# irconde/SSL4POLYP

Hardware: AMD Instinct MI355X
Metric: training-step images/sec/node, ViT-B/16 224^2 (cls fine-tune) (higher is better)
Workload: dtype bf16; 1 GPU; ViT-B/16 classification fine-tune, bs=64/GPU, 224^2, AdamW, random init, finetune mode full (finetune.py:49-91); global_batch=64, parallelism=dp1, launch=eager, lr_schedule=constant

## Files before the change

include/polypmae.h:

```cpp
#ifndef POLYPMAE_H
#define POLYPMAE_H
#include <stddef.h>
#include <stdint.h>

#ifdef __cplusplus
extern "C" {
#endif

enum pm_status { PM_OK = 0, PM_EINVAL = -1, PM_ESHAPE = -2, PM_EARCH = -3, PM_ELAUNCH = -4, PM_EALIGN = -5 };
enum pm_dtype { PM_F32 = 0, PM_BF16 = 1, PM_F16 = 2 };

enum pm_epilogue {
  PM_EPI_STORE = 0,
  PM_EPI_GELU = 1,
  PM_EPI_RESIDUAL = 2,
  PM_EPI_DGELU = 3,
  PM_EPI_ACCUM = 4
};

const char* pm_strerror(int status);
int pm_abi_version(void);

int pm_layernorm_fwd(const float* x, long ldx, const float* gamma, const float* beta, void* y, int out_dtype,
                     float* mean, float* rstd, int M, int D, float eps, void* stream);
// ... 172 lines not shown
                            size_t ws_bytes, void* stream);

typedef struct pm_block_fwd_desc {
  const float* x;
  float* x_mid;
  float* x_out;
  void* ln1;
  float* mean1;
  float* rstd1;
  void* qkv;
  float* lse;
  void* attn;
  void* ln2;
  float* mean2;
  float* rstd2;
  void* h_pre;
  void* h_act;
  const float *norm1_w, *norm1_b, *norm2_w, *norm2_b;
  const void *qkv_w, *proj_w, *fc1_w, *fc2_w;
  const float *qkv_b, *proj_b, *fc1_b, *fc2_b;
  int rows, samples, N, D, Hd, heads;
  int dtype;
  int gemm_variant;
  float eps;
} pm_block_fwd_desc;
int pm_vit_block_fwd(const pm_block_fwd_desc* d, void* stream);

typedef struct pm_block_bwd_desc {
  const float* x_in;
  const float* x_mid;
  const void *ln1, *qkv, *attn, *ln2, *h_pre, *h_act;
  const float *mean1, *rstd1, *mean2, *rstd2, *lse;
  const float *norm1_w, *norm2_w;
  const void *qkv_w, *proj_w, *fc1_w, *fc2_w;
  const float* dx;
  const void* dx_act;
  float* dmid;
  void* dmid_act;
  float* din;
  void* din_act;
  void *d_hidden, *d_qkv, *d_ln, *d_attn;
  float* delta;
  float *g_norm1_w, *g_norm1_b, *g_norm2_w, *g_norm2_b;
  float *g_qkv_w, *g_proj_w, *g_fc1_w, *g_fc2_w;
  float *g_qkv_b, *g_proj_b, *g_fc1_b, *g_below_bias;
  void* ws_ln;
  size_t ws_ln_bytes;
  void* ws_group;
  size_t ws_group_bytes;
  void *side_stream, *ev_join, *ev_fork, *ev_done;
  int samples, N, D, Hd, heads, dtype, gemm_variant, group_blocks, accumulate;
  int two_groups;
  void *side_stream2, *ev_fork2, *ev_done2;
} pm_block_bwd_desc;
int pm_vit_block_bwd(const pm_block_bwd_desc* d, void* stream);

int pm_vit_head_fwd(const float* x, int N, int pool, const float* gamma, const float* beta, const float* W,
                    const float* bias, float* feat, float* xhat_mean, float* mean, float* rstd, float* logits, int B, int D,
                    int n_class, float eps, void* stream);
int pm_vit_head_bwd(const float* dlogits, const float* dfeat, const float* x, int N, int pool, const float* gamma,
                    const float* W, const float* feat, const float* xhat_mean, const float* mean, const float* rstd,
                    float* dx, void* dx_act, int act_dtype, float* dW, float* dbias, float* dgamma, float* dbeta, int B,
                    int D, int n_class, void* stream);
int pm_cls_head_fwd(const float* x, int N, const float* gamma, const float* beta, const float* W, const float* bias,
                    float* xn, float* mean, float* rstd, float* logits, int B, int D, int n_class, float eps,
                    void* stream);
int pm_cls_head_bwd(const float* dlogits, const float* x, int N, const float* gamma, const float* W, const float* xn,
                    const float* mean, const float* rstd, float* dx, void* dx_act, int act_dtype, float* dW,
                    float* dbias, float* dgamma, float* dbeta, int B, int D, int n_class, void* stream);

int pm_supervised_loss_fwd(const float* logits, const long long* targets, const float* pos_weight,
                           const float* class_weights, float* loss, float* dlogits, int B, int n_class, void* stream);
int pm_scale(const float* x, const float* scale, float* out, long n, void* stream);

int pm_dgelu(const void* dy, const void* pre, void* out, int dtype, long n, void* stream);

int pm_adamw(float* p, const float* g, float* m, float* v, void* shadow, int shadow_dtype, long n, float lr,
             float beta1, float beta2, float eps, float weight_decay, int step, float grad_scale, void* stream);

int pm_adamw_tick(float* hyper, int n_groups, void* stream);
int pm_adamw_dev(float* p, const float* g, float* m, float* v, void* shadow, int shadow_dtype, long n,
                 const float* hyper, void* stream);

int pm_loss_scale_update(float* state, const float* stats, float* hyper, int n_groups, float growth_factor,
                         float backoff_factor, int growth_interval, void* stream);

int pm_grad_stats(const float* g, long n, float* out, void* stream);

enum pm_ws_kind { PM_WS_LAYERNORM_BWD = 1, PM_WS_COLSUM = 2, PM_WS_UNSHUFFLE_BWD = 4 };
size_t pm_gemm_workspace_bytes(int a_kmajor, int b_kmajor, int in_dtype, int M, int N, int K, const pm_gemm_opts* opts);
size_t pm_workspace_bytes(int kind, int M, int N);

typedef struct pm_comm pm_comm;
int pm_comm_unique_id(void* id128);
int pm_comm_create(pm_comm** out, const void* id128, int rank, int world);
int pm_comm_world(const pm_comm* c, int* rank, int* world);
int pm_comm_allreduce_f32(pm_comm* c, float* base, const long* lo, const long* hi, int n_buckets, void* stream);
int pm_comm_destroy(pm_comm* c);

int pm_boot_metrics_workspace(int N, int M, int R, int K, int C, size_t* bytes);
int pm_boot_metrics(const double* score, const int* order, const unsigned char* label, const int* cluster, const int* draws,
                    const double* tau, double* out, int N, int M, int R, int K, int C, int sorted_ready, void* workspace,
                    size_t ws_bytes, void* stream);

int pm_select_tau_workspace(int N, int M, size_t* bytes);
int pm_select_tau(const double* score, const int* order, const unsigned char* label, const double* previous_tau, int policy,
                  double* out, double* candidates, int N, int M, void* workspace, size_t ws_bytes, void* stream);

#ifdef __cplusplus
}
#endif
#endif
```

ssl4polyp_amd/_lib.py:

```python
from __future__ import annotations

import ctypes
import os
from ctypes import c_char_p, c_float, c_int, c_long, c_void_p

PM_F32, PM_BF16, PM_F16 = 0, 1, 2
EPI_STORE, EPI_GELU, EPI_RESIDUAL, EPI_DGELU, EPI_ACCUM = 0, 1, 2, 3, 4

_HERE = os.path.dirname(os.path.abspath(__file__))
LIB_PATH = os.environ.get("POLYPMAE_LIB") or os.path.join(_HERE, "lib", "libpolypmae.so")

P, I, L, F = c_void_p, c_int, c_long, c_float

SIGNATURES = {
    "pm_layernorm_fwd": [P, L, P, P, P, I, P, P, I, I, F, P],
    "pm_layernorm_bwd": [P, I, P, L, P, P, P, P, L, P, L, P, I, P, P, P, I, I, P, ctypes.c_size_t, P],
    "pm_vit_block_fwd": [P, P],
    "pm_vit_block_bwd": [P, P],
    "pm_gemm": [P, L, I, P, L, I, I, P, P, L, I, I, P, P, I, I, I, P],
    "pm_gemm_ws": [P, L, I, P, L, I, I, P, P, L, I, I, P, P, I, I, I, P, ctypes.c_size_t, P],
    "pm_gemm_ex": [P, L, I, P, L, I, I, P, P, L, I, I, P, P, I, I, I, P, ctypes.c_size_t, P, P],
    "pm_wgrad_group": [P, I, I, I, I, P, ctypes.c_size_t, P],
    "pm_wgrad_group_plan": [P, I, I, I, P, P, P],
    "pm_gemm_plan": [I, I, I, I, I, I, I, I, I, I, ctypes.c_size_t, P, P],
    "pm_attention_plan": [I, I, I, I, I, I, P],
    "pm_attention_fwd": [P, P, P, I, I, I, I, I, P],
    "pm_attention_bwd": [P, P, P, P, P, P, I, I, I, I, I, P],
    "pm_colsum": [P, L, I, P, I, I, P],
    "pm_colsum_ws": [P, L, I, P, I, I, P, ctypes.c_size_t, P],
    "pm_patch_im2col": [P, P, P, L, I, I, I, I, I, I, P],
    "pm_pad_cast": [P, L, P, L, I, I, I, I, I, P],
    "pm_unpad_add": [P, L, P, L, I, I, I, P],
    "pm_assemble_tokens": [P, P, P, P, P, I, I, I, P],
    "pm_assemble_tokens_bwd": [P, P, P, I, P, P, I, I, I, P],
    "pm_mae_noise": [P, L, ctypes.c_ulonglong, ctypes.c_uint, P],
    "pm_mae_masking": [P, P, P, P, I, I, I, P],
    "pm_mae_unshuffle": [P, P, P, P, P, I, I, I, I, P],
    "pm_mae_unshuffle_bwd": [P, P, P, I, P, I, I, I, I, P, ctypes.c_size_t, P],
    "pm_mae_loss_fwd": [P, P, L, I, P, I, I, I, I, I, P],
    "pm_mae_loss_finish": [P, P, L, P, P, P],
    "pm_mae_loss_bwd": [P, P, L, I, P, P, P, P, L, I, I, I, I, I, I, P],
    "pm_cast": [P, P, I, L, P],
    "pm_gather_rows": [P, L, P, P, I, L, P],
    "pm_scatter_rows_zero": [P, P, P, I, L, P],
    "pm_preprocess_u8": [P, P, P, I, I, I, F, F, F, F, F, F, P],
    "pm_aug_resize_u8": [P, P, P, P, P, I, P, P, I, I, I, I, I, I, P],
    "pm_aug_resized_crop_u8": [P, P, P, I, I, I, I, I, P, ctypes.c_size_t, P],
    "pm_aug_resized_crop_ragged_u8": [P, P, P, P, P, I, I, I, I, I, P, ctypes.c_size_t, P],
    "pm_aug_color_jitter_u8": [P, P, P, P, I, I, I, P],
    "pm_aug_gaussian_blur_u8": [P, P, P, P, I, I, I, I, P],
    "pm_aug_geometry_u8": [P, P, P, I, I, I, I, F, F, F, F, F, F, P],
    "pm_aug_pil_gaussian_blur_u8": [P, P, P, P, I, I, I, I, P],
    "pm_aug_occlude_u8": [P, P, I, I, I, P],
    "pm_aug_jpeg_roundtrip_u8": [P, P, P, I, I, I, P],
    "pm_jpeg_decode": [P, L, P, I, P, I, P, I, P, I, P, L, P, I, P, P, L, L, P, L, P],
    "pm_jpeg_decode_parallel": [P, L, P, I, P, I, P, I, P, I, P, L, P, I, P, P, L, L, P, L, P, I, I, P, ctypes.c_size_t, P, P],
    "pm_jpeg_decode_workspace": [I, I, P],
    "pm_jpeg_decode_planes": [P, L, P, I, P, I, P, I, P, I, P, P, L, P, I, I, P, ctypes.c_size_t, P, P],
    "pm_jpeg_resized_crop_workspace": [I, I, I, I, P],
    "pm_jpeg_resized_crop_u8": [P, L, P, I, P, L, P, I, P, P, P, P, I, I, I, I, I, P, ctypes.c_size_t, P],
    "pm_comm_unique_id": [P],
    "pm_comm_create": [P, P, I, I],
    "pm_comm_world": [P, P, P],
    "pm_comm_allreduce_f32": [P, P, P, P, I, P],
    "pm_comm_destroy": [P],
    "pm_vit_head_fwd": [P, I, I, P, P, P, P, P, P, P, P, P, I, I, I, F, P],
    "pm_vit_head_bwd": [P, P, P, I, I, P, P, P, P, P, P, P, P, I, P, P, P, P, I, I, I, P],
    "pm_supervised_loss_fwd": [P, P, P, P, P, P, I, I, P],
    "pm_scale": [P, P, P, L, P],
    "pm_cls_head_fwd": [P, I, P, P, P, P, P, P, P, P, I, I, I, F, P],
    "pm_cls_head_bwd": [P, P, I, P, P, P, P, P, P, P, I, P, P, P, P, I, I, I, P],
    "pm_adamw": [P, P, P, P, P, I, L, F, F, F, F, F, I, F, P],
    "pm_adamw_tick": [P, I, P],
    "pm_adamw_dev": [P, P, P, P, P, I, L, P, P],
    "pm_grad_stats": [P, L, P, P],
    "pm_loss_scale_update": [P, P, P, I, F, F, I, P],
    "pm_dgelu": [P, P, P, I, L, P],
    "pm_boot_metrics_workspace": [I, I, I, I, I, P],
    "pm_boot_metrics": [P, P, P, P, P, P, P, I, I, I, I, I, I, P, ctypes.c_size_t, P],
    "pm_select_tau_workspace": [I, I, P],
    "pm_select_tau": [P, P, P, P, I, P, P, I, I, P, ctypes.c_size_t, P],
}

ABI_VERSION = 16
PM_GROUP_WHOLE_K = -1

WS_LAYERNORM_BWD, WS_COLSUM, WS_UNSHUFFLE_BWD = 1, 2, 4


class GemmPlanInfo(ctypes.Structure):
    _fields_ = [("family", c_int), ("cfg", c_int), ("tile_m", c_int), ("tile_n", c_int), ("split_k", c_int), ("band", c_int),
                ("ws_bytes", ctypes.c_size_t)]


GEMM_GENERIC, GEMM_LDS128, GEMM_RING, GEMM_RING_WGRAD = 0, 1, 2, 3


class AttentionPlanInfo(ctypes.Structure):
    _fields_ = [("family", c_int), ("nt", c_int), ("ct", c_int), ("grid", c_int), ("launches", c_int),
                ("lds_bytes", ctypes.c_size_t * 2)]


ATTN_FWD_HEAD, ATTN_FWD_PERSISTENT, ATTN_BWD_SPLIT, ATTN_BWD_FUSED = 0, 1, 2, 3


class GemmOpts(ctypes.Structure):
    _fields_ = [("max_blocks", c_int), ("variant", c_int)]


class WgradItem(ctypes.Structure):
    _fields_ = [("dY", c_void_p), ("lddy", c_long), ("X", c_void_p), ("ldx", c_long), ("dW", c_void_p), ("lddw", c_long),
                ("n_out", c_int), ("n_in", c_int), ("accumulate", c_int), ("dbias", c_void_p)]


class BlockBwdDesc(ctypes.Structure):
    _fields_ = ([(n, c_void_p) for n in ("x_in", "x_mid", "ln1", "qkv", "attn", "ln2", "h_pre", "h_act", "mean1", "rstd1", "mean2",
                                        "rstd2", "lse", "norm1_w", "norm2_w", "qkv_w", "proj_w", "fc1_w", "fc2_w", "dx", "dx_act",
                                        "dmid", "dmid_act", "din", "din_act", "d_hidden", "d_qkv", "d_ln", "d_attn", "delta",
                                        "g_norm1_w", "g_norm1_b", "g_norm2_w", "g_norm2_b", "g_qkv_w", "g_proj_w", "g_fc1_w",
                                        "g_fc2_w", "g_qkv_b", "g_proj_b", "g_fc1_b", "g_below_bias")] +
                [("ws_ln", c_void_p), ("ws_ln_bytes", ctypes.c_size_t), ("ws_group", c_void_p), ("ws_group_bytes", ctypes.c_size_t)] +
                [(n, c_void_p) for n in ("side_stream", "ev_join", "ev_fork", "ev_done")] +
                [(n, c_int) for n in ("samples", "N", "D", "Hd", "heads", "dtype", "gemm_variant", "group_blocks", "accumulate",
                                      "two_groups")] +
                [(n, c_void_p) for n in ("side_stream2", "ev_fork2", "ev_done2")])


class BlockFwdDesc(ctypes.Structure):
    _fields_ = ([(n, c_void_p) for n in ("x", "x_mid", "x_out", "ln1", "mean1", "rstd1", "qkv", "lse", "attn", "ln2", "mean2",
                                        "rstd2", "h_pre", "h_act", "norm1_w", "norm1_b", "norm2_w", "norm2_b", "qkv_w", "proj_w",
                                        "fc1_w", "fc2_w", "qkv_b", "proj_b", "fc1_b", "fc2_b")] +
                [(n, c_int) for n in ("rows", "samples", "N", "D", "Hd", "heads", "dtype", "gemm_variant")] +
                [("eps", ctypes.c_float)])


PM_EINVAL, PM_ESHAPE, PM_EALIGN = -1, -2, -5
_lib = None


class PolypMaeError(RuntimeError):
    pass


def load():
    global _lib
    if _lib is not None:
        return _lib
    if not os.path.exists(LIB_PATH):
        raise PolypMaeError(
            f"{LIB_PATH} not found: build it with `python -c 'import __graft_entry__ as g; g.build()'`. "
            "There is no CPU/eager fallback for the MI355X hot path.")
    lib = ctypes.CDLL(LIB_PATH)
    lib.pm_strerror.restype = c_char_p
    lib.pm_strerror.argtypes = [c_int]
    lib.pm_abi_version.restype = c_int
    lib.pm_abi_version.argtypes = []
    if lib.pm_abi_version() != ABI_VERSION:
        raise PolypMaeError(f"{LIB_PATH} has ABI version {lib.pm_abi_version()}, this package binds version {ABI_VERSION}: "
                            "rebuild with `python -c 'import __graft_entry__ as g; g.build(force=True)'`")
    lib.pm_gemm_workspace_bytes.restype = ctypes.c_size_t
    lib.pm_gemm_workspace_bytes.argtypes = [I, I, I, I, I, I, P]
    lib.pm_workspace_bytes.restype = ctypes.c_size_t
    lib.pm_workspace_bytes.argtypes = [I, I, I]
    lib.pm_aug_resized_crop_workspace_bytes.restype = ctypes.c_size_t
    lib.pm_aug_resized_crop_workspace_bytes.argtypes = [I, I, I, I]
    lib.pm_wgrad_group_workspace_bytes.restype = ctypes.c_size_t
    lib.pm_wgrad_group_workspace_bytes.argtypes = [P, I, I, I]
    for name, argtypes in SIGNATURES.items():
        fn = getattr(lib, name)
        fn.restype = c_int
        fn.argtypes = argtypes
    _lib = lib
    return lib


def check(status: int, what: str) -> None:
    if status != 0:
        raise PolypMaeError(f"{what} failed: {load().pm_strerror(status).decode()} (status {status})")


def dtype_code(torch_dtype) -> int:
    import torch

    if torch_dtype == torch.float32:
        return PM_F32
    if torch_dtype == torch.bfloat16:
        return PM_BF16
    if torch_dtype == torch.float16:
        return PM_F16
    raise PolypMaeError(f"unsupported dtype {torch_dtype}")
```

ssl4polyp_amd/csrc/pm_misc.hip:

```cpp
#include "pm_common.h"

namespace {

template <typename T>
__global__ __launch_bounds__(256) void colsum_kernel(const T* __restrict__ x, long ldx, float* __restrict__ out,
                                                     float* __restrict__ partials, int M, int N) {
  const int lane = threadIdx.x & 63, wave = threadIdx.x >> 6;
  const int n = blockIdx.x * 256 + lane * 4;
  f32x4 acc = {0.f, 0.f, 0.f, 0.f};
  if (n < N) {
    for (long m = (long)blockIdx.y * 4 + wave; m < M; m += (long)gridDim.y * 4) acc += load4<T>(x + m * ldx + n);
  }
  block_colsum_tail(acc, out, partials, N);
}

template <typename T>
__global__ __launch_bounds__(256) void im2col_kernel(const float* __restrict__ imgs, const int* __restrict__ ids_keep,
                                                     T* __restrict__ cols, long ldcols, int C, int img, int p, int keep) {
  const int b = blockIdx.x / keep, j = blockIdx.x % keep;
  const int grid = img / p;
  const int pid = ids_keep ? ids_keep[b * keep + j] : j;
  const int gy = pid / grid, gx = pid % grid;
  const float* src = imgs + (long)b * C * img * img + (long)gy * p * img + gx * p;
  T* dst = cols + (long)blockIdx.x * ldcols;
// ... 118 lines not shown
                                                            int B, int H, int W, f32x4 mean, f32x4 stdv) {
  const int w4 = W >> 2;
  const long total = (long)B * H * w4;
  for (long id = (long)blockIdx.x * 256 + threadIdx.x; id < total; id += (long)gridDim.x * 256) {
    const int xq = id % w4;
    const int y = (id / w4) % H;
    const int b = id / ((long)w4 * H);
    const int f = flags ? flags[b] : 0;
    const int sy = (f & 2) ? H - 1 - y : y;
    const unsigned char* row = src + ((long)b * H + sy) * W * 3;
    float px[4][3];
#pragma unroll
    for (int i = 0; i < 4; ++i) {
      const int x = xq * 4 + i;
      const int sx = (f & 1) ? W - 1 - x : x;
#pragma unroll
      for (int c = 0; c < 3; ++c) px[i][c] = (float)row[sx * 3 + c];
    }
#pragma unroll
    for (int c = 0; c < 3; ++c) {
      f32x4 v;
#pragma unroll
      for (int i = 0; i < 4; ++i) v[i] = __fdiv_rn(__fdiv_rn(px[i][c], 255.0f) - mean[c], stdv[c]);
      *reinterpret_cast<f32x4*>(dst + (((long)b * 3 + c) * H + y) * W + xq * 4) = v;
    }
  }
}

template <typename T>
__global__ __launch_bounds__(256) void cast_kernel(const float* __restrict__ src, T* __restrict__ dst, long n) {
  const long nvec = n >> 2;
  for (long i = (long)blockIdx.x * 256 + threadIdx.x; i < nvec; i += (long)gridDim.x * 256)
    store4<T>(dst + 4 * i, *reinterpret_cast<const f32x4*>(src + 4 * i));
  if (blockIdx.x == 0 && threadIdx.x < (n & 3)) dst[(nvec << 2) + threadIdx.x] = (T)src[(nvec << 2) + threadIdx.x];
}

template <typename T>
__global__ __launch_bounds__(256) void dgelu_kernel(const T* __restrict__ dy, const T* __restrict__ pre, T* __restrict__ out, long n) {
  const long nvec = n >> 2;
  for (long i = (long)blockIdx.x * 256 + threadIdx.x; i < nvec; i += (long)gridDim.x * 256)
    store4<T>(out + 4 * i, load4<T>(dy + 4 * i) * gelu_act_grad4<T>(load4<T>(pre + 4 * i)));
}

template <typename T>
__global__ __launch_bounds__(256) void adamw_kernel(float* __restrict__ p, const float* __restrict__ g, float* __restrict__ m,
                                                    float* __restrict__ v, T* __restrict__ shadow, long n, float lr,
                                                    float beta1, float beta2, float eps, float wd, float bc1, float rsqrt_bc2,
                                                    float gscale) {
  const long nvec = n >> 2;
  for (long i = (long)blockIdx.x * 256 + threadIdx.x; i < nvec; i += (long)gridDim.x * 256) {
    f32x4 pp = *reinterpret_cast<const f32x4*>(p + 4 * i);
    const f32x4 gg = *reinterpret_cast<const f32x4*>(g + 4 * i);
    f32x4 mm = *reinterpret_cast<const f32x4*>(m + 4 * i);
    f32x4 vv = *reinterpret_cast<const f32x4*>(v + 4 * i);
#pragma unroll
    for (int e = 0; e < 4; ++e) {
      const float gr = gg[e] * gscale;
      pp[e] *= (1.0f - lr * wd);
      mm[e] = beta1 * mm[e] + (1.0f - beta1) * gr;
      vv[e] = beta2 * vv[e] + (1.0f - beta2) * gr * gr;
      const float denom = sqrtf(vv[e]) * rsqrt_bc2 + eps;
      pp[e] -= (lr / bc1) * (mm[e] / denom);
    }
    *reinterpret_cast<f32x4*>(p + 4 * i) = pp;
    *reinterpret_cast<f32x4*>(m + 4 * i) = mm;
    *reinterpret_cast<f32x4*>(v + 4 * i) = vv;
    if (shadow) store4<T>(shadow + 4 * i, pp);
  }
}


constexpr int kHyperStride = 16;
__global__ void adamw_tick_kernel(float* __restrict__ hyper, int n_groups) {
  const int g = blockIdx.x * blockDim.x + threadIdx.x;
  if (g >= n_groups) return;
  float* h = hyper + (long)g * kHyperStride;
  if (h[9] != 0.f) return;
  const float step = h[6] + 1.0f;
  h[6] = step;
  h[7] = (float)(1.0 - pow((double)h[1], (double)step));
  h[8] = (float)(1.0 / sqrt(1.0 - pow((double)h[2], (double)step)));
}

template <typename T>
__global__ __launch_bounds__(256) void adamw_dev_kernel(float* __restrict__ p, const float* __restrict__ g, float* __restrict__ m,
                                                        float* __restrict__ v, T* __restrict__ shadow, long n,
                                                        const float* __restrict__ hyper) {
  if (hyper[9] != 0.f) return;
  const float lr = hyper[0], beta1 = hyper[1], beta2 = hyper[2], eps = hyper[3], wd = hyper[4];
  const float gscale = hyper[5] * (hyper[10] != 0.f ? hyper[10] : 1.0f);
  const float bc1 = hyper[7], rsqrt_bc2 = hyper[8];
  const long nvec = n >> 2;
  for (long i = (long)blockIdx.x * 256 + threadIdx.x; i < nvec; i += (long)gridDim.x * 256) {
    f32x4 pp = *reinterpret_cast<const f32x4*>(p + 4 * i);
    const f32x4 gg = *reinterpret_cast<const f32x4*>(g + 4 * i);
    f32x4 mm = *reinterpret_cast<const f32x4*>(m + 4 * i);
    f32x4 vv = *reinterpret_cast<const f32x4*>(v + 4 * i);
#pragma unroll
    for (int e = 0; e < 4; ++e) {
      const float gr = gg[e] * gscale;
      pp[e] *= (1.0f - lr * wd);
      mm[e] = beta1 * mm[e] + (1.0f - beta1) * gr;
      vv[e] = beta2 * vv[e] + (1.0f - beta2) * gr * gr;
      const float denom = sqrtf(vv[e]) * rsqrt_bc2 + eps;
      pp[e] -= (lr / bc1) * (mm[e] / denom);
    }
    *reinterpret_cast<f32x4*>(p + 4 * i) = pp;
    *reinterpret_cast<f32x4*>(m + 4 * i) = mm;
    *reinterpret_cast<f32x4*>(v + 4 * i) = vv;
    if (shadow) store4<T>(shadow + 4 * i, pp);
  }
}

__global__ __launch_bounds__(256) void grad_stats_kernel(const float* __restrict__ g, long n, float* __restrict__ out) {
  __shared__ float red[3][4];
  float ss = 0.f, nn = 0.f, ni = 0.f;
  const long nvec = n >> 2;
  for (long i = (long)blockIdx.x * 256 + threadIdx.x; i < nvec; i += (long)gridDim.x * 256) {
    const f32x4 v = *reinterpret_cast<const f32x4*>(g + 4 * i);
#pragma unroll
    for (int e = 0; e < 4; ++e) {
      ss += v[e] * v[e];
      nn += (v[e] != v[e]) ? 1.f : 0.f;
      ni += (fabsf(v[e]) == INFINITY) ? 1.f : 0.f;
    }
  }
  if (blockIdx.x == 0 && threadIdx.x < (n & 3)) {
    const float v = g[(nvec << 2) + threadIdx.x];
    ss += v * v;
    nn += (v != v) ? 1.f : 0.f;
    ni += (fabsf(v) == INFINITY) ? 1.f : 0.f;
  }
  ss = wave_sum(ss);
  nn = wave_sum(nn);
  ni = wave_sum(ni);
  const int lane = threadIdx.x & 63, wave = threadIdx.x >> 6;
  if (lane == 0) {
    red[0][wave] = ss;
    red[1][wave] = nn;
    red[2][wave] = ni;
  }
  __syncthreads();
  if (threadIdx.x < 3) {
    const int k = threadIdx.x;
    atomicAdd(out + k, (red[k][0] + red[k][1]) + (red[k][2] + red[k][3]));
  }
}

__global__ void loss_scale_update_kernel(float* __restrict__ state, const float* __restrict__ stats, float* __restrict__ hyper,
                                         int n_groups, float growth, float backoff, int interval) {
  const float scale = state[0];
  const float found = (stats[1] + stats[2]) > 0.f ? 1.f : 0.f;
  const float tracker = state[1];
  __syncthreads();
  for (int g = threadIdx.x; g < n_groups; g += blockDim.x) {
    hyper[(long)g * kHyperStride + 9] = found;
    hyper[(long)g * kHyperStride + 10] = 1.0f / scale;
  }
  if (threadIdx.x == 0) {
    state[2] = found;
    state[4] += 1.f;
    state[5] = 1.0f / scale;
    if (found != 0.f) {
      state[0] = scale * backoff;
      state[1] = 0.f;
      state[3] += 1.f;
    } else {
      const float t = tracker + 1.f;
      if (t >= (float)interval) {
        state[0] = scale * growth;
        state[1] = 0.f;
      } else {
        state[1] = t;
      }
    }
  }
}

__global__ __launch_bounds__(256) void gather_rows_kernel(const unsigned int* __restrict__ src, long ld_words, const int* __restrict__ idx,
                                                          unsigned int* __restrict__ dst, int R, long words) {
  const long total = (long)R * words;
  for (long i = (long)blockIdx.x * 256 + threadIdx.x; i < total; i += (long)gridDim.x * 256) {
    const int r = i / words;
    const long w = i % words;
    dst[i] = src[(long)idx[r] * ld_words + w];
  }
}
__global__ __launch_bounds__(256) void scatter_rows_zero_kernel(const u32x4* __restrict__ src, const int* __restrict__ inv,
                                                                u32x4* __restrict__ dst, int M, long vecs) {
  const long total = (long)M * vecs;
  for (long i = (long)blockIdx.x * 256 + threadIdx.x; i < total; i += (long)gridDim.x * 256) {
    const int m = i / vecs;
    const long v = i % vecs;
// ... 75 lines not shown
                                                   (T*)demb, dpos, B, keep, D));
  if (dcls)
    hipLaunchKernelGGL(cls_grad_kernel, dim3((D + 63) / 64), dim3(256), 0, pm_stream(stream), dx, dcls, dpos, B,
                       (long)(keep + 1) * D, D);
  return pm_check_launch();
}

extern "C" int pm_preprocess_u8(const unsigned char* src, const unsigned char* flip_flags, float* dst, int B, int H, int W,
                                float mean_r, float mean_g, float mean_b, float std_r, float std_g, float std_b,
                                void* stream) {
  if (!src || !dst) return PM_EINVAL;
  if (B <= 0 || H <= 0 || W <= 0 || (W & 3)) return PM_ESHAPE;
  if (((uintptr_t)dst & 15)) return PM_EALIGN;
  if (!(std_r > 0.f) || !(std_g > 0.f) || !(std_b > 0.f)) return PM_EINVAL;
  const long total = (long)B * H * (W >> 2);
  const dim3 grid(cap_grid(total, 256, 8192));
  hipLaunchKernelGGL(preprocess_u8_kernel, grid, dim3(256), 0, pm_stream(stream), src, flip_flags, dst, B, H, W,
                     f32x4{mean_r, mean_g, mean_b, 0.f}, f32x4{std_r, std_g, std_b, 1.f});
  return pm_check_launch();
}

extern "C" int pm_cast(const float* src, void* dst, int dst_dtype, long n, void* stream) {
  if (!src || !dst) return PM_EINVAL;
  if (n <= 0) return PM_ESHAPE;
  if (((uintptr_t)src & 15) || ((uintptr_t)dst & 7)) return PM_EALIGN;
  const dim3 grid(cap_grid(n >> 2, 256, 4096));
  PM_DISPATCH_ACT(dst_dtype, T, hipLaunchKernelGGL(cast_kernel<T>, grid, dim3(256), 0, pm_stream(stream), src, (T*)dst, n));
  return pm_check_launch();
}

extern "C" int pm_gather_rows(const void* src, long ld_bytes, const int* idx, void* dst, int R, long row_bytes, void* stream) {
  if (!src || !idx || !dst) return PM_EINVAL;
  if (R <= 0 || row_bytes <= 0 || ld_bytes < row_bytes) return PM_ESHAPE;
  if ((row_bytes & 3) || (ld_bytes & 3) || ((uintptr_t)src & 3) || ((uintptr_t)dst & 3)) return PM_EALIGN;
  const long total = (long)R * (row_bytes >> 2);
  hipLaunchKernelGGL(gather_rows_kernel, dim3(cap_grid(total, 256, 4096)), dim3(256), 0, pm_stream(stream), (const unsigned int*)src,
                     ld_bytes >> 2, idx, (unsigned int*)dst, R, row_bytes >> 2);
  return pm_check_launch();
}

extern "C" int pm_scatter_rows_zero(const void* src, const int* inv, void* dst, int M, long row_bytes, void* stream) {
  if (!src || !inv || !dst) return PM_EINVAL;
  if (M <= 0 || row_bytes <= 0) return PM_ESHAPE;
  if ((row_bytes & 15) || ((uintptr_t)src & 15) || ((uintptr_t)dst & 15)) return PM_EALIGN;
  const long total = (long)M * (row_bytes >> 4);
  hipLaunchKernelGGL(scatter_rows_zero_kernel, dim3(cap_grid(total, 256, 8192)), dim3(256), 0, pm_stream(stream), (const u32x4*)src, inv,
                     (u32x4*)dst, M, row_bytes >> 4);
  return pm_check_launch();
}

extern "C" int pm_dgelu(const void* dy, const void* pre, void* out, int dtype, long n, void* stream) {
  if (!dy || !pre || !out) return PM_EINVAL;
  if (n <= 0 || (n & 3)) return PM_ESHAPE;
  if (((uintptr_t)dy & 7) || ((uintptr_t)pre & 7) || ((uintptr_t)out & 7)) return PM_EALIGN;
  const dim3 grid(cap_grid(n >> 2, 256, 4096));
  PM_DISPATCH_ACT(dtype, T, hipLaunchKernelGGL(dgelu_kernel<T>, grid, dim3(256), 0, pm_stream(stream), (const T*)dy, (const T*)pre,
                                               (T*)out, n));
  return pm_check_launch();
}

extern "C" int pm_adamw(float* p, const float* g, float* m, float* v, void* shadow, int shadow_dtype, long n, float lr,
                        float beta1, float beta2, float eps, float weight_decay, int step, float grad_scale,
                        void* stream) {
  if (!p || !g || !m || !v) return PM_EINVAL;
  if (n <= 0 || (n & 3) || step < 1) return PM_ESHAPE;
  const double bc1 = 1.0 - pow((double)beta1, (double)step);
  const double bc2 = 1.0 - pow((double)beta2, (double)step);
  const float rsqrt_bc2 = (float)(1.0 / sqrt(bc2));
  const dim3 grid(cap_grid(n >> 2, 256, 4096));
  if (!shadow) shadow_dtype = PM_BF16;
  PM_DISPATCH_ACT(shadow_dtype, T, hipLaunchKernelGGL(adamw_kernel<T>, grid, dim3(256), 0, pm_stream(stream), p, g, m, v, (T*)shadow, n,
                                                      lr, beta1, beta2, eps, weight_decay, (float)bc1, rsqrt_bc2, grad_scale));
  return pm_check_launch();
}


extern "C" int pm_adamw_tick(float* hyper, int n_groups, void* stream) {
  if (!hyper) return PM_EINVAL;
  if (n_groups <= 0) return PM_ESHAPE;
  hipLaunchKernelGGL(adamw_tick_kernel, dim3((n_groups + 63) / 64), dim3(64), 0, pm_stream(stream), hyper, n_groups);
  return pm_check_launch();
}

extern "C" int pm_adamw_dev(float* p, const float* g, float* m, float* v, void* shadow, int shadow_dtype, long n,
                            const float* hyper, void* stream) {
  if (!p || !g || !m || !v || !hyper) return PM_EINVAL;
  if (n <= 0 || (n & 3)) return PM_ESHAPE;
  const dim3 grid(cap_grid(n >> 2, 256, 4096));
  if (!shadow) shadow_dtype = PM_BF16;
  PM_DISPATCH_ACT(shadow_dtype, T, hipLaunchKernelGGL(adamw_dev_kernel<T>, grid, dim3(256), 0, pm_stream(stream), p, g, m, v, (T*)shadow,
                                                      n, hyper));
  return pm_check_launch();
}

extern "C" int pm_loss_scale_update(float* state, const float* stats, float* hyper, int n_groups, float growth_factor,
                                    float backoff_factor, int growth_interval, void* stream) {
  if (!state || !stats || !hyper) return PM_EINVAL;
  if (n_groups <= 0 || growth_interval <= 0 || !(growth_factor >= 1.f) || !(backoff_factor > 0.f && backoff_factor <= 1.f)) return PM_ESHAPE;
  hipLaunchKernelGGL(loss_scale_update_kernel, dim3(1), dim3(64), 0, pm_stream(stream), state, stats, hyper, n_groups,
                     growth_factor, backoff_factor, growth_interval);
  return pm_check_launch();
}

extern "C" int pm_grad_stats(const float* g, long n, float* out, void* stream) {
  if (!g || !out) return PM_EINVAL;
  if (n <= 0) return PM_ESHAPE;
  if ((uintptr_t)g & 15) return PM_EALIGN;
  hipLaunchKernelGGL(grad_stats_kernel, dim3(cap_grid(n >> 2, 256, 1024)), dim3(256), 0, pm_stream(stream), g, n, out);
  return pm_check_launch();
}

extern "C" const char* pm_strerror(int status) {
  switch (status) {
    case PM_OK: return "ok";
    case PM_EINVAL: return "invalid argument (null pointer / unknown dtype or epilogue)";
    case PM_ESHAPE: return "unsupported shape";
    case PM_EARCH: return "no gfx950 device";
    case PM_ELAUNCH: return "kernel launch failed";
    case PM_EALIGN: return "pointer / leading dimension not 16-byte aligned";
    default: return "unknown status";
  }
}

extern "C" int pm_abi_version(void) { return 16; }

extern "C" size_t pm_workspace_bytes(int kind, int M, int N) {
  if (M <= 0 || N <= 0) return 0;
  switch (kind) {
    case PM_WS_LAYERNORM_BWD: {
      long g = (M + 3) / 4;
      if (g > 1024) g = 1024;
      if (g < 64) g = 64;
      return (size_t)g * 3 * N * sizeof(float);
    }
    case PM_WS_COLSUM: return (size_t)cap_grid(M, 64, 128) * N * sizeof(float);
    case PM_WS_UNSHUFFLE_BWD: return (size_t)1024 * N * sizeof(float);
    default: return 0;
  }
}
```

ssl4polyp_amd/optim.py:

```python
from __future__ import annotations

from typing import Dict, Iterable, List, Optional

import contextlib

import torch

from . import _lib
from .engine import _ptr, _stream


def add_weight_decay(model, weight_decay=1e-5, skip_list=()):
    decay, no_decay = [], []
    for name, param in model.named_parameters():
        if not param.requires_grad:
            continue
        if len(param.shape) == 1 or name.endswith(".bias") or name in skip_list:
            no_decay.append(param)
        else:
            decay.append(param)
    return [{"params": no_decay, "weight_decay": 0.0}, {"params": decay, "weight_decay": weight_decay}]


class FusedAdamW(torch.optim.Optimizer):
# ... 45 lines not shown
        segs = []
        for r, lo, hi in items:
            if segs and segs[-1][0] == r and segs[-1][2] == lo:
                segs[-1] = (r, segs[-1][1], hi)
            else:
                segs.append((r, lo, hi))
        return segs

    HYPER_STRIDE = 16

    def _host_hyper(self):
        rows = []
        for group in self.param_groups:
            b1, b2 = group["betas"]
            rows.append((float(group["lr"]), float(b1), float(b2), float(group["eps"]), float(group["weight_decay"]),
                         float(self.grad_scale)))
        return rows

    def sync_hyper(self, force: bool = False):
        f = self._ensure_state()
        rows = self._host_hyper()
        if getattr(self, "_hyper", None) is None or self._hyper.device != f.device:
            self._hyper = torch.zeros(len(rows), self.HYPER_STRIDE, dtype=torch.float32, device=f.device)
            for gi, group in enumerate(self.param_groups):
                self._hyper[gi, 6] = float(group.get("step", 0))
            self._hyper_host = None
        if force or rows != self._hyper_host:
            if f.device.type == "cuda":
                if getattr(self, "_hyper_pin", None) is None or self._hyper_pin[0].shape[0] != len(rows):
                    self._hyper_pin = [torch.empty(len(rows), 6, dtype=torch.float32).pin_memory() for _ in range(4)]
                    self._hyper_pin_ev = [None] * 4
                    self._hyper_slot = 0
                i = self._hyper_slot
                self._hyper_slot = (i + 1) % 4
                if self._hyper_pin_ev[i] is not None:
                    self._hyper_pin_ev[i].synchronize()
                self._hyper_pin[i].copy_(torch.tensor(rows, dtype=torch.float32))
                self._hyper[:, :6].copy_(self._hyper_pin[i], non_blocking=True)
                ev = torch.cuda.Event()
                ev.record(torch.cuda.current_stream(f.device))
                self._hyper_pin_ev[i] = ev
            else:
                self._hyper[:, :6].copy_(torch.tensor(rows, dtype=torch.float32))
            self._hyper_host = rows

    @torch.no_grad()
    def step(self, closure=None, loss_scaler: "Optional[LossScaler]" = None):
        loss = None
        if closure is not None:
            with torch.enable_grad():
                loss = closure()
        f = self._ensure_state()
        rt = self._rt
        rt.wait_updates()
        if self.grad_sync is not None:
            self.grad_sync.wait()
        capturing = f.device.type == "cuda" and torch.cuda.is_current_stream_capturing()
        if not capturing or getattr(self, "_hyper", None) is None:
            self.sync_hyper()
        lib = self._rt.k.lib
        overlap = self.overlap_forward and not capturing and f.device.type == "cuda"
        work = []
        for gi, group in enumerate(self.param_groups):
            group["step"] = int(group.get("step", 0)) + 1
            for r, lo, hi in self._segments(f, group):
                work.append((gi, r, lo, hi))
        scaled = loss_scaler is not None and loss_scaler.enabled
        stat_segs = [(r, lo, hi) for _, r, lo, hi in work] if scaled else []
        if not scaled and getattr(self, "_scaler_used", False):
            self._hyper[:, 9:11] = 0.0
            self._scaler_used = False
        if overlap:
            cuts = sorted(f.offset[i] for i, n in enumerate(f.names) if n.endswith("attn.qkv.weight"))
            split = []
            for gi, r, lo, hi in work:
                if r != "mat":
                    split.append((gi, r, lo, hi))
                    continue
                pts = [lo] + [c for c in cuts if lo < c < hi] + [hi]
                split += [(gi, r, a, b) for a, b in zip(pts[:-1], pts[1:])]
            work = sorted(split, key=lambda w: (w[1] != "vec", w[2]))
            main = torch.cuda.current_stream(f.device)
            side = rt.k.side_stream(f.device)
            ev = torch.cuda.Event()
            ev.record(main)
            side.wait_event(ev)
            stream_ctx = torch.cuda.stream(side)
        else:
            stream_ctx = contextlib.nullcontext()
        with stream_ctx:
            if scaled:
                state, stats = loss_scaler._device_state(f.device)
                stats.zero_()
                for r, lo, hi in stat_segs:
                    _lib.check(lib.pm_grad_stats(_ptr(f.G[r][lo:hi]), hi - lo, _ptr(stats), _stream()), "pm_grad_stats")
                _lib.check(lib.pm_loss_scale_update(_ptr(state), _ptr(stats), _ptr(self._hyper), len(self.param_groups),
                                                    loss_scaler.growth_factor, loss_scaler.backoff_factor,
                                                    loss_scaler.growth_interval, _stream()), "pm_loss_scale_update")
                self._scaler_used = True
            _lib.check(lib.pm_adamw_tick(_ptr(self._hyper), len(self.param_groups), _stream()), "pm_adamw_tick")
            for gi, r, lo, hi in work:
                shadow = f.S[lo:hi] if (r == "mat" and f.S is not None) else None
                _lib.check(lib.pm_adamw_dev(_ptr(f.P[r][lo:hi]), _ptr(f.G[r][lo:hi]), _ptr(self._M[r][lo:hi]),
                                            _ptr(self._V[r][lo:hi]), _ptr(shadow),
                                            _lib.dtype_code(shadow.dtype) if shadow is not None else 0, hi - lo,
                                            _ptr(self._hyper[gi]), _stream()), "pm_adamw_dev")
                if overlap:
                    done = torch.cuda.Event()
                    done.record(side)
                    rt.pending_updates.append((r, lo, hi, done))
        return loss

    def sync(self) -> None:
        self._rt.wait_updates()

    def grad_stats(self) -> torch.Tensor:
        f = self._ensure_state()
        self._rt.wait_updates()
        out = torch.zeros(3, dtype=torch.float32, device=f.device)
        lib = self._rt.k.lib
        for group in self.param_groups:
            for r, lo, hi in self._segments(f, group):
                _lib.check(lib.pm_grad_stats(_ptr(f.G[r][lo:hi]), hi - lo, _ptr(out), _stream()), "pm_grad_stats")
        return out

    def state_dict(self, host: bool = False):
        self._rt.wait_updates()
        f = self._rt.flat
        idx = {id(p): i for i, p in enumerate(f.params)} if f is not None else {}
        state, groups, k = {}, [], 0
        M, V = self._M, self._V
        if host and M:
            M = {r: t.detach().cpu() for r, t in M.items()}
            V = {r: t.detach().cpu() for r, t in V.items()}
        for group in self.param_groups:
            ids = []
            for p in group["params"]:
                i = idx.get(id(p))
                if i is not None and M:
                    r, lo, n = f.region[i], f.offset[i], f.numel[i]
                    state[k] = {"step": torch.tensor(float(group.get("step", 0))),
                                "exp_avg": M[r][lo:lo + n].view(p.shape).clone(),
                                "exp_avg_sq": V[r][lo:lo + n].view(p.shape).clone()}
                ids.append(k)
                k += 1
            g = {kk: v for kk, v in group.items() if kk != "params"}
            g["params"] = ids
            groups.append(g)
        return {"state": state, "param_groups": groups}

    def load_state_dict(self, sd):
        f = self._ensure_state()
        self._rt.wait_updates()
        idx = {id(p): i for i, p in enumerate(f.params)}
        for group, saved in zip(self.param_groups, sd["param_groups"]):
            for kk, v in saved.items():
                if kk != "params":
                    group[kk] = v
            for p, k in zip(group["params"], saved["params"]):
                st = sd["state"].get(k)
                if st is None:
                    continue
                i = idx[id(p)]
                r, lo, n = f.region[i], f.offset[i], f.numel[i]
                self._M[r][lo:lo + n].copy_(st["exp_avg"].reshape(-1))
                self._V[r][lo:lo + n].copy_(st["exp_avg_sq"].reshape(-1))
                group["step"] = int(float(st["step"]))
        self._hyper = None


class _ScaleLossFn(torch.autograd.Function):

    @staticmethod
    def forward(ctx, loss, scale):
        lib = _lib.load()
        x = loss.reshape(1).contiguous().float()
        out = torch.empty_like(x)
        _lib.check(lib.pm_scale(_ptr(x), _ptr(scale), _ptr(out), 1, _stream()), "pm_scale")
        ctx.scale = scale
        return out.reshape(())

    @staticmethod
    def backward(ctx, dout):
        lib = _lib.load()
        d = dout.reshape(1).contiguous().float()
        out = torch.empty_like(d)
        _lib.check(lib.pm_scale(_ptr(d), _ptr(ctx.scale), _ptr(out), 1, _stream()), "pm_scale")
        return out.reshape(()), None


class LossScaler:

    def __init__(self, init_scale: float = 65536.0, growth_factor: float = 2.0, backoff_factor: float = 0.5,
                 growth_interval: int = 2000, enabled: bool = True):
# ... 75 lines not shown
```

Baseline: 6332 images/sec.

## Batch overlapped AdamW segment launches into one native call with cached descriptors

Adds pm_adamw_segments, which performs the stream wait, the hyperparameter tick, every per-segment AdamW launch and the done-event records in a single C call. The segment descriptor array and events are cached on the Python side so the per-step ctypes and event-creation work goes away. The AdamW kernel is also restructured to process chunks of four vectors per thread with nontemporal loads and stores, and the overlapped path caps the grid at 256 blocks so it leaves compute units free for the concurrent main-stream work. Reusing events and cached pointers risks stale state if the buffers move, though the cache key includes the data pointers.

```diff
diff --git a/include/polypmae.h b/include/polypmae.h
--- a/include/polypmae.h
+++ b/include/polypmae.h
@@ -278,6 +278,20 @@
 int pm_adamw_dev(float* p, const float* g, float* m, float* v, void* shadow, int shadow_dtype, long n,
                  const float* hyper, void* stream);
 
+typedef struct pm_adamw_segment {
+  float* p;
+  const float* g;
+  float *m, *v;
+  void* shadow;
+  int shadow_dtype;
+  long n;
+  const float* hyper;
+  void* done_event;
+} pm_adamw_segment;
+int pm_adamw_segments(const pm_adamw_segment* segs, int n_segs, float* hyper, int n_groups, void* wait_event, void* stream,
+                      int max_blocks);
+int pm_adamw_grid(long n, int max_blocks);
+
 int pm_loss_scale_update(float* state, const float* stats, float* hyper, int n_groups, float growth_factor,
                          float backoff_factor, int growth_interval, void* stream);
 
diff --git a/ssl4polyp_amd/_lib.py b/ssl4polyp_amd/_lib.py
--- a/ssl4polyp_amd/_lib.py
+++ b/ssl4polyp_amd/_lib.py
@@ -73,6 +73,8 @@
     "pm_adamw": [P, P, P, P, P, I, L, F, F, F, F, F, I, F, P],
     "pm_adamw_tick": [P, I, P],
     "pm_adamw_dev": [P, P, P, P, P, I, L, P, P],
+    "pm_adamw_segments": [P, I, P, I, P, P, I],
+    "pm_adamw_grid": [L, I],
     "pm_grad_stats": [P, L, P, P],
     "pm_loss_scale_update": [P, P, P, I, F, F, I, P],
     "pm_dgelu": [P, P, P, I, L, P],
@@ -111,6 +113,11 @@
 class WgradItem(ctypes.Structure):
     _fields_ = [("dY", c_void_p), ("lddy", c_long), ("X", c_void_p), ("ldx", c_long), ("dW", c_void_p), ("lddw", c_long),
                 ("n_out", c_int), ("n_in", c_int), ("accumulate", c_int), ("dbias", c_void_p)]
+
+
+class AdamwSegment(ctypes.Structure):
+    _fields_ = [("p", c_void_p), ("g", c_void_p), ("m", c_void_p), ("v", c_void_p), ("shadow", c_void_p), ("shadow_dtype", c_int),
+                ("n", c_long), ("hyper", c_void_p), ("done_event", c_void_p)]
 
 
 class BlockBwdDesc(ctypes.Structure):
diff --git a/ssl4polyp_amd/csrc/pm_misc.hip b/ssl4polyp_amd/csrc/pm_misc.hip
--- a/ssl4polyp_amd/csrc/pm_misc.hip
+++ b/ssl4polyp_amd/csrc/pm_misc.hip
@@ -224,33 +224,65 @@
   h[8] = (float)(1.0 / sqrt(1.0 - pow((double)h[2], (double)step)));
 }
 
+constexpr int kAdamwUnroll = 4;
+constexpr int kAdamwChunk = kAdamwUnroll * 256;
+
+struct AdamwHyper {
+  float lr, beta1, beta2, eps, wd, gscale, bc1, rsqrt_bc2;
+};
+
+__device__ __forceinline__ f32x4 ld_stream(const float* a) { return __builtin_nontemporal_load(reinterpret_cast<const f32x4*>(a)); }
+__device__ __forceinline__ void st_stream(float* a, f32x4 x) { __builtin_nontemporal_store(x, reinterpret_cast<f32x4*>(a)); }
+
+template <typename T>
+__device__ __forceinline__ void adamw_dev_vec(float* __restrict__ p, float* __restrict__ m, float* __restrict__ v, T* __restrict__ shadow,
+                                              long i, f32x4 pp, const f32x4 gg, f32x4 mm, f32x4 vv, const AdamwHyper& h) {
+  const float lr = h.lr, beta1 = h.beta1, beta2 = h.beta2, eps = h.eps, wd = h.wd, gscale = h.gscale;
+  const float bc1 = h.bc1, rsqrt_bc2 = h.rsqrt_bc2;
+#pragma unroll
+  for (int e = 0; e < 4; ++e) {
+    const float gr = gg[e] * gscale;
+    pp[e] *= (1.0f - lr * wd);
+    mm[e] = beta1 * mm[e] + (1.0f - beta1) * gr;
+    vv[e] = beta2 * vv[e] + (1.0f - beta2) * gr * gr;
+    const float denom = sqrtf(vv[e]) * rsqrt_bc2 + eps;
+    pp[e] -= (lr / bc1) * (mm[e] / denom);
+  }
+  st_stream(p + 4 * i, pp);
+  st_stream(m + 4 * i, mm);
+  st_stream(v + 4 * i, vv);
+  if (shadow) store4<T>(shadow + 4 * i, pp);
+}
+
 template <typename T>
 __global__ __launch_bounds__(256) void adamw_dev_kernel(float* __restrict__ p, const float* __restrict__ g, float* __restrict__ m,
                                                         float* __restrict__ v, T* __restrict__ shadow, long n,
                                                         const float* __restrict__ hyper) {
   if (hyper[9] != 0.f) return;
-  const float lr = hyper[0], beta1 = hyper[1], beta2 = hyper[2], eps = hyper[3], wd = hyper[4];
-  const float gscale = hyper[5] * (hyper[10] != 0.f ? hyper[10] : 1.0f);
-  const float bc1 = hyper[7], rsqrt_bc2 = hyper[8];
+  AdamwHyper h;
+  h.lr = hyper[0], h.beta1 = hyper[1], h.beta2 = hyper[2], h.eps = hyper[3], h.wd = hyper[4];
+  h.gscale = hyper[5] * (hyper[10] != 0.f ? hyper[10] : 1.0f);
+  h.bc1 = hyper[7], h.rsqrt_bc2 = hyper[8];
   const long nvec = n >> 2;
-  for (long i = (long)blockIdx.x * 256 + threadIdx.x; i < nvec; i += (long)gridDim.x * 256) {
-    f32x4 pp = *reinterpret_cast<const f32x4*>(p + 4 * i);
-    const f32x4 gg = *reinterpret_cast<const f32x4*>(g + 4 * i);
-    f32x4 mm = *reinterpret_cast<const f32x4*>(m + 4 * i);
-    f32x4 vv = *reinterpret_cast<const f32x4*>(v + 4 * i);
-#pragma unroll
-    for (int e = 0; e < 4; ++e) {
-      const float gr = gg[e] * gscale;
-      pp[e] *= (1.0f - lr * wd);
-      mm[e] = beta1 * mm[e] + (1.0f - beta1) * gr;
-      vv[e] = beta2 * vv[e] + (1.0f - beta2) * gr * gr;
-      const float denom = sqrtf(vv[e]) * rsqrt_bc2 + eps;
-      pp[e] -= (lr / bc1) * (mm[e] / denom);
-    }
-    *reinterpret_cast<f32x4*>(p + 4 * i) = pp;
-    *reinterpret_cast<f32x4*>(m + 4 * i) = mm;
-    *reinterpret_cast<f32x4*>(v + 4 * i) = vv;
-    if (shadow) store4<T>(shadow + 4 * i, pp);
+  for (long c = (long)blockIdx.x * kAdamwChunk; c < nvec; c += (long)gridDim.x * kAdamwChunk) {
+    const long i0 = c + threadIdx.x;
+    if (c + kAdamwChunk <= nvec) {
+      f32x4 pp[kAdamwUnroll], gg[kAdamwUnroll], mm[kAdamwUnroll], vv[kAdamwUnroll];
+#pragma unroll
+      for (int k = 0; k < kAdamwUnroll; ++k) {
+        const long i = i0 + k * 256;
+        pp[k] = ld_stream(p + 4 * i);
+        gg[k] = ld_stream(g + 4 * i);
+        mm[k] = ld_stream(m + 4 * i);
+        vv[k] = ld_stream(v + 4 * i);
+      }
+#pragma unroll
+      for (int k = 0; k < kAdamwUnroll; ++k) adamw_dev_vec<T>(p, m, v, shadow, i0 + k * 256, pp[k], gg[k], mm[k], vv[k], h);
+    } else {
+      for (long i = i0; i < nvec; i += 256)
+        adamw_dev_vec<T>(p, m, v, shadow, i, ld_stream(p + 4 * i), ld_stream(g + 4 * i),
+                         ld_stream(m + 4 * i), ld_stream(v + 4 * i), h);
+    }
   }
 }
 
@@ -492,15 +524,55 @@
   return pm_check_launch();
 }
 
-extern "C" int pm_adamw_dev(float* p, const float* g, float* m, float* v, void* shadow, int shadow_dtype, long n,
-                            const float* hyper, void* stream) {
+extern "C" int pm_adamw_grid(long n, int max_blocks) {
+  if (n <= 0 || (n & 3) || max_blocks < 0) return PM_ESHAPE;
+  return max_blocks == 0 ? cap_grid(n >> 2, 256, 4096) : cap_grid(n >> 2, kAdamwChunk, max_blocks);
+}
+
+static int adamw_dev_check(const float* p, const float* g, const float* m, const float* v, const void* shadow, int shadow_dtype,
+                           long n, const float* hyper) {
   if (!p || !g || !m || !v || !hyper) return PM_EINVAL;
   if (n <= 0 || (n & 3)) return PM_ESHAPE;
-  const dim3 grid(cap_grid(n >> 2, 256, 4096));
+  if (shadow && shadow_dtype != PM_BF16 && shadow_dtype != PM_F16 && shadow_dtype != PM_F32) return PM_EINVAL;
+  return PM_OK;
+}
+
+static int adamw_dev_launch(float* p, const float* g, float* m, float* v, void* shadow, int shadow_dtype, long n, const float* hyper,
+                            int max_blocks, void* stream) {
+  const dim3 grid(pm_adamw_grid(n, max_blocks));
   if (!shadow) shadow_dtype = PM_BF16;
   PM_DISPATCH_ACT(shadow_dtype, T, hipLaunchKernelGGL(adamw_dev_kernel<T>, grid, dim3(256), 0, pm_stream(stream), p, g, m, v, (T*)shadow,
                                                       n, hyper));
   return pm_check_launch();
+}
+
+extern "C" int pm_adamw_dev(float* p, const float* g, float* m, float* v, void* shadow, int shadow_dtype, long n,
+                            const float* hyper, void* stream) {
+  const int st = adamw_dev_check(p, g, m, v, shadow, shadow_dtype, n, hyper);
+  if (st != PM_OK) return st;
+  return adamw_dev_launch(p, g, m, v, shadow, shadow_dtype, n, hyper, 0, stream);
+}
+
+extern "C" int pm_adamw_segments(const pm_adamw_segment* segs, int n_segs, float* hyper, int n_groups, void* wait_event, void* stream,
+                                 int max_blocks) {
+  if (!segs || !hyper) return PM_EINVAL;
+  if (n_segs <= 0 || n_groups <= 0 || max_blocks < 0) return PM_ESHAPE;
+  for (int i = 0; i < n_segs; ++i) {
+    const pm_adamw_segment& s = segs[i];
+    const int st = adamw_dev_check(s.p, s.g, s.m, s.v, s.shadow, s.shadow_dtype, s.n, s.hyper);
+    if (st != PM_OK) return st;
+  }
+  hipStream_t q = pm_stream(stream);
+  if (wait_event && hipStreamWaitEvent(q, (hipEvent_t)wait_event, 0) != hipSuccess) return PM_ELAUNCH;
+  int st = pm_adamw_tick(hyper, n_groups, stream);
+  if (st != PM_OK) return st;
+  for (int i = 0; i < n_segs; ++i) {
+    const pm_adamw_segment& s = segs[i];
+    st = adamw_dev_launch(s.p, s.g, s.m, s.v, s.shadow, s.shadow_dtype, s.n, s.hyper, max_blocks, stream);
+    if (st != PM_OK) return st;
+    if (s.done_event && hipEventRecord((hipEvent_t)s.done_event, q) != hipSuccess) return PM_ELAUNCH;
+  }
+  return PM_OK;
 }
 
 extern "C" int pm_loss_scale_update(float* state, const float* stats, float* hyper, int n_groups, float growth_factor,
diff --git a/ssl4polyp_amd/optim.py b/ssl4polyp_amd/optim.py
--- a/ssl4polyp_amd/optim.py
+++ b/ssl4polyp_amd/optim.py
@@ -151,9 +151,10 @@
             work = sorted(split, key=lambda w: (w[1] != "vec", w[2]))
             main = torch.cuda.current_stream(f.device)
             side = rt.k.side_stream(f.device)
-            ev = torch.cuda.Event()
+            ev = self._event(-1, side)
             ev.record(main)
-            side.wait_event(ev)
+            if scaled or not work:
+                side.wait_event(ev)
             stream_ctx = torch.cuda.stream(side)
         else:
             stream_ctx = contextlib.nullcontext()
@@ -167,6 +168,13 @@
                                                     loss_scaler.growth_factor, loss_scaler.backoff_factor,
                                                     loss_scaler.growth_interval, _stream()), "pm_loss_scale_update")
                 self._scaler_used = True
+            if overlap and work:
+                segs, events = self._segment_array(f, work, side)
+                _lib.check(lib.pm_adamw_segments(segs, len(work), _ptr(self._hyper), len(self.param_groups),
+                                                 None if scaled else ev.cuda_event, _stream(), self.OVERLAP_MAX_BLOCKS),
+                           "pm_adamw_segments")
+                rt.pending_updates += [(r, lo, hi, done) for (_, r, lo, hi), done in zip(work, events)]
+                return loss
             _lib.check(lib.pm_adamw_tick(_ptr(self._hyper), len(self.param_groups), _stream()), "pm_adamw_tick")
             for gi, r, lo, hi in work:
                 shadow = f.S[lo:hi] if (r == "mat" and f.S is not None) else None
@@ -174,11 +182,32 @@
                                             _ptr(self._V[r][lo:hi]), _ptr(shadow),
                                             _lib.dtype_code(shadow.dtype) if shadow is not None else 0, hi - lo,
                                             _ptr(self._hyper[gi]), _stream()), "pm_adamw_dev")
-                if overlap:
-                    done = torch.cuda.Event()
-                    done.record(side)
-                    rt.pending_updates.append((r, lo, hi, done))
         return loss
+
+    OVERLAP_MAX_BLOCKS = 256
+
+    def _event(self, i, side):
+        cache = self.__dict__.setdefault("_events", {})
+        e = cache.get(i)
+        if e is None:
+            e = cache[i] = torch.cuda.Event()
+            e.record(side)
+        return e
+
+    def _segment_array(self, f, work, side):
+        S = f.S
+        key = (tuple(work), S.dtype if S is not None else None, self._hyper.data_ptr(), _ptr(S)) + \
+            tuple(t[r].data_ptr() for r in ("mat", "vec") for t in (f.P, f.G, self._M, self._V))
+        if getattr(self, "_seg_key", None) != key:
+            events = [self._event(i, side) for i in range(len(work))]
+            segs = (_lib.AdamwSegment * len(work))()
+            for i, (gi, r, lo, hi) in enumerate(work):
+                shadow = S[lo:hi] if (r == "mat" and S is not None) else None
+                segs[i] = _lib.AdamwSegment(_ptr(f.P[r][lo:hi]), _ptr(f.G[r][lo:hi]), _ptr(self._M[r][lo:hi]), _ptr(self._V[r][lo:hi]),
+                                            _ptr(shadow), _lib.dtype_code(shadow.dtype) if shadow is not None else 0, hi - lo,
+                                            _ptr(self._hyper[gi]), events[i].cuda_event)
+            self._seg_key, self._seg_args = key, (segs, events)
+        return self._seg_args
 
     def sync(self) -> None:
         self._rt.wait_updates()
```

New measurement: 6403 images/sec (median of 6 runs). 1.01x the previous value.
